# DJNing/articulated-object-nerf

Measured on AMD Instinct MI355X. Metric: rays/sec at 640×480×(64c+128f) samples; PSNR vs reference, higher is better.
Workload: dtype f16x3 (fp16 hi/lo split MFMA, fp32 accumulate)

## Files before the change

### articulated-object-nerf_amd/aonerf/_lib.py

```python
import ctypes
import os

import torch

_HERE = os.path.dirname(os.path.abspath(__file__))
LIB_PATH = os.path.join(os.path.dirname(_HERE), "lib", "libaonerf.so")

c_i64, c_int, c_float, c_size, vp = ctypes.c_int64, ctypes.c_int, ctypes.c_float, ctypes.c_size_t, ctypes.c_void_p

PREC = {"fp32": 0, "f16x3": 1}
PREC_F16X3_TRAIN = 4
PREC_BF16 = 2
ACT_NONE, ACT_VANILLA, ACT_ARTIC = 0, 1, 2
OPACITY = {None: 0, "mse": 1, "ce": 2, "autorf": 3}


class AonMlpParams(ctypes.Structure):
    _fields_ = [("pts_w", vp * 8), ("pts_b", vp * 8), ("density_w", vp), ("density_b", vp),
                ("bottleneck_w", vp), ("bottleneck_b", vp), ("views_w", vp), ("views_b", vp),
                ("rgb_w", vp), ("rgb_b", vp), ("w_rows", c_i64 * 12), ("w_cols", c_i64 * 12),
                ("b_len", c_i64 * 12)]


class AonMlpArtParams(ctypes.Structure):
# ... 123 lines not shown
    "aon_pos_enc": (c_int, [vp, c_i64, c_int, c_int, vp, vp]),
    "aon_sample_rays": (c_int, [vp, vp, c_int, c_i64, c_int, c_int, c_float, vp, c_i64, c_int,
                                c_float, vp, vp, vp, vp, vp]),
    "aon_cast_rays": (c_int, [vp, vp, vp, c_i64, c_int, vp, c_i64, vp, c_int, c_int, vp, vp]),
    "aon_cast_rays_tiled": (c_int, [vp, vp, vp, c_i64, c_int, c_int, c_int, c_int, vp, vp]),
    "aon_sample_pdf": (c_int, [vp, c_i64, vp, c_i64, c_i64, c_int, c_int, vp, c_i64, vp, c_int,
                               vp, vp, vp, vp, vp]),
    "aon_composite_march": (c_int, [vp, vp, vp, c_i64, c_int, c_int, c_int, vp, c_i64, c_int, vp,
                                    vp, vp, vp, vp, vp]),
    "aon_mlp_packed_bytes": (c_size, [c_int]),
    "aon_mlp_read_status": (c_int, [vp, c_size, ctypes.POINTER(ctypes.c_uint32), vp]),
    "aon_mlp_pack": (c_int, [ctypes.POINTER(AonMlpParams), c_int, vp, vp]),
    "aon_mlp_fwd": (c_int, [vp, c_int, vp, vp, vp, vp, c_i64, c_int, c_int, vp, vp]),
    "aon_mlp_fwd_encoded": (c_int, [vp, c_int, vp, vp, c_i64, c_int, c_int, vp, vp]),
    "aon_mlp_fwd_sigma": (c_int, [vp, c_int, vp, vp, vp, c_i64, c_int, c_int, vp, vp]),
    "aon_mlp_fwd_cond": (c_int, [vp, c_int, vp, vp, vp, vp, c_i64, c_int, c_int, vp, vp]),
    "aon_mlp_fwd_train": (c_int, [vp, vp, vp, vp, vp, c_i64, c_int, vp, vp, vp, vp, vp, vp, vp]),
    "aon_mlp_fwd_train_bf16": (c_int, [vp, vp, vp, vp, vp, c_i64, c_int, vp, vp, vp, vp, vp, vp,
                                       vp, vp]),
    "aon_mlp_bwd_pack_bf16": (c_int, [ctypes.POINTER(AonMlpParams), vp, vp]),
    "aon_mlp_bwd_bf16": (c_int, [vp, vp, vp, c_i64, vp, vp, vp, vp, vp]),
    "aon_relu_masks": (c_int, [vp, c_i64, c_int, vp, vp]),
    "aon_absmax": (c_int, [vp, c_i64, vp, vp]),
    "aon_mlp_bwd_packed_bytes": (c_size, []),
    "aon_mlp_bwd_pack": (c_int, [ctypes.POINTER(AonMlpParams), vp, vp]),
    "aon_mlp_bwd": (c_int, [vp, vp, vp, c_i64, vp, vp, vp, vp, vp]),
    "aon_mlp_art_packed_bytes": (c_size, []),
    "aon_mlp_art_pack": (c_int, [ctypes.POINTER(AonMlpArtParams), vp, vp]),
    "aon_mlp_art_fwd": (c_int, [vp, vp, vp, vp, vp, c_i64, c_int, c_int, vp, vp]),
    "aon_mlp_art_fwd_points": (c_int, [vp, vp, vp, c_i64, c_int, c_int, vp, vp]),
# ... 196 lines not shown
```

### articulated-object-nerf_amd/aonerf/model.py

```python
import warnings

import torch
import torch.nn as nn
import torch.nn.init as init

from . import _lib as L
from . import helper
from .numerics import resolve as _resolve_numerics

_DEFAULT_GEOMETRY = dict(min_deg_point=0, max_deg_point=10, deg_view=4, netdepth=8, netwidth=256,
                         netdepth_condition=1, netwidth_condition=128, skip_layer=4, input_ch=3,
                         input_ch_view=3, num_rgb_channels=3, num_density_channels=1)


class NeRFMLP(nn.Module):

    def __init__(self, min_deg_point, max_deg_point, deg_view, netdepth: int = 8,
                 netwidth: int = 256, netdepth_condition: int = 1, netwidth_condition: int = 128,
                 skip_layer: int = 4, input_ch: int = 3, input_ch_view: int = 3,
                 num_rgb_channels: int = 3, num_density_channels: int = 1,
                 precision: str = "f16x3"):
        super().__init__()
        self.min_deg_point, self.max_deg_point, self.deg_view = min_deg_point, max_deg_point, deg_view
        self.netdepth, self.netwidth, self.skip_layer = netdepth, netwidth, skip_layer
# ... 61 lines not shown
        L.require_gpu(rays_o, rays_d, viewdirs, t_vals, cond)
        B, S = t_vals.shape
        raw = torch.empty((B * S, 4), device=t_vals.device)
        if cond is not None:
            if tuple(cond.shape) != (B, 27):
                raise ValueError("forward_rays expects cond (B, 27)")
            L.call("aon_mlp_fwd_cond", L.ptr(self.packed_weights()), L.PREC[self.precision],
                   L.ptr(L.contig(rays_o)), L.ptr(L.contig(rays_d)), L.ptr(L.contig(cond)),
                   L.ptr(L.contig(t_vals)), B, S, act, L.ptr(raw), L.stream(t_vals.device))
            return raw
        L.call("aon_mlp_fwd", L.ptr(self.packed_weights()), L.PREC[self.precision],
               L.ptr(L.contig(rays_o)), L.ptr(L.contig(rays_d)), L.ptr(L.contig(viewdirs)),
               L.ptr(L.contig(t_vals)), B, S, act, L.ptr(raw), L.stream(t_vals.device))
        return raw

    def forward_sigma(self, rays_o, rays_d, t_vals, act=L.ACT_NONE):
        L.require_gpu(rays_o, rays_d, t_vals)
        B, S = t_vals.shape
        raw = torch.empty((B * S, 4), device=t_vals.device)
        L.call("aon_mlp_fwd_sigma", L.ptr(self.packed_weights()), L.PREC[self.precision],
               L.ptr(L.contig(rays_o)), L.ptr(L.contig(rays_d)), L.ptr(L.contig(t_vals)), B, S, act,
               L.ptr(raw), L.stream(t_vals.device))
        return raw

    def forward(self, x, condition):
        L.require_gpu(x, condition)
        B, S, C = x.shape
        if C != 63 or tuple(condition.shape) != (B, 27):
            raise ValueError("NeRFMLP.forward expects x (B, S, 63) and condition (B, 27)")
        raw = torch.empty((B * S, 4), device=x.device)
        L.call("aon_mlp_fwd_encoded", L.ptr(self.packed_weights()), L.PREC[self.precision],
               L.ptr(L.contig(x)), L.ptr(L.contig(condition)), B, S, L.ACT_NONE, L.ptr(raw),
               L.stream(x.device))
        raw = raw.view(B, S, 4)
        return raw[..., :3], raw[..., 3:]


# ... 19 lines not shown


def composite_march(raw, t_vals, d, white_bkgd, act, u, u_stride, num_fine_samples,
                    keep_weights):
    B, S = t_vals.shape
    dev = t_vals.device
    comp = torch.empty((B, 3), device=dev)
    acc = torch.empty((B,), device=dev)
    depth = torch.empty((B,), device=dev)
    weights = torch.empty((B, S), device=dev) if keep_weights else None
    t_fine = torch.empty((B, S + num_fine_samples), device=dev)
    L.call("aon_composite_march", L.ptr(raw), L.ptr(t_vals), L.ptr(d), B, S, int(bool(white_bkgd)),
           act, L.ptr(u), u_stride, num_fine_samples, L.ptr(comp), L.ptr(acc), L.ptr(weights),
           L.ptr(depth), L.ptr(t_fine), L.stream(dev))
    return (comp, acc, depth, weights), t_fine


def march_ok(S, num_fine_samples, fused=True):
    return fused and 3 <= S <= 256 and 1 <= num_fine_samples <= 256


def level_t_vals(level, o, d, t_prev, w_prev, randomized, near, far, num_coarse_samples,
                 num_fine_samples, lindisp, u_coarse=None, u_fine=None):
    dev = o.device
    B = o.shape[0]
    if level == 0:
        t_vals, _ = helper.sample_along_rays(o, d, num_coarse_samples, near, far, randomized,
                                             lindisp, u=u_coarse, want_coords=False)
        return t_vals
    Sc = t_prev.shape[1]
# ... 69 lines not shown
                comp, acc, depth, weights = RenderLevel.apply(o, d, v, t_vals, bool(white_bkgd),
                                                              noise, token, cfg, timers, *params)
                out = (comp, acc, depth, weights) if return_weights else (comp, acc, depth)
                if return_intermediates:
                    out = out + (dict(t_vals=t_vals, weights=weights),)
                ret.append(out)
                continue
            keep_w = level == 0 or return_weights or return_intermediates
            march = level == 0 and march_ok(S, self.num_fine_samples, self.fused_march)
            if march:
                keep_w = return_weights or return_intermediates
            with torch.no_grad():
                out, weights, t_next = self._render_level_fused(
                    mlp, o, d, v, t_vals, randomized, white_bkgd, level, timers, keep_w,
                    sigma_only=two_pass and level == 0, cond=cond if level == 1 else None,
                    march_u=(lambda: fine_uniforms(B, self.num_fine_samples, randomized, dev,
                                                   u_fine)) if march else None)
            if not return_weights:
                out = out[:3] + out[4:]
            if not return_intermediates:
                out = out[:4] if return_weights else out[:3]
            ret.append(None if fine_only and level == 0 else out)
        if (not training and self.range_check and self.coarse_mlp.precision.startswith("f16x3")
                and not torch.cuda.is_current_stream_capturing()
                and L.range_overflow([self.coarse_mlp._packed, self.fine_mlp._packed])):
            warnings.warn("NeRF: an MLP activation exceeded the fp16x3 range; re-rendered with "
                          "precision='fp32'", RuntimeWarning)
            prec = self.coarse_mlp.precision
            self.set_precision("fp32")
            if rng is not None:
# ... 1 lines not shown
            try:
                return self.forward(rays, randomized, white_bkgd, near, far, u_coarse=u_coarse,
                                    u_fine=u_fine, return_weights=return_weights,
                                    return_intermediates=return_intermediates, timers=timers,
                                    fine_only=fine_only)
            finally:
                self.set_precision(prec)
        return ret

    def _level_t(self, level, o, d, t_prev, w_prev, randomized, near, far, u_coarse, u_fine):
        return level_t_vals(level, o, d, t_prev, w_prev, randomized, near, far,
                            self.num_coarse_samples, self.num_fine_samples, self.lindisp,
                            u_coarse, u_fine)

    def _render_level_fused(self, mlp, o, d, v, t_vals, randomized, white_bkgd, level, timers,
                            keep_weights=True, march_u=None, sigma_only=False, cond=None):
        B, S = t_vals.shape
        dev = o.device
        noisy = self.noise_std > 0 and randomized
        ev = _events(timers)
        act = L.ACT_NONE if noisy else L.ACT_VANILLA
        if sigma_only:
            raw = mlp.forward_sigma(o, d, t_vals, act=act)
        else:
            raw = mlp.forward_rays(o, d, v, t_vals, act=act, cond=cond)
        _record(timers, ev, f"mlp{level}", B * S)
        if noisy:
            raw[:, 3] += torch.rand_like(raw[:, 3]) * self.noise_std
        act = L.ACT_VANILLA if noisy else L.ACT_NONE
        t_next = None
        ev = _events(timers)
        if march_u is not None:
            u, u_stride = march_u()
            (comp, acc, depth, weights), t_next = composite_march(
                raw, t_vals, d, white_bkgd, act, u, u_stride, self.num_fine_samples, keep_weights)
            _record(timers, ev, f"march{level}", B * S)
# ... 11 lines not shown
```

### articulated-object-nerf_amd/csrc/composite_core.hpp

```cpp
#pragma once

#include "aon_common.hpp"
#include "torch_sum.hpp"

namespace aon {

#ifndef AON_COMP_OCC_FINE
#define AON_COMP_OCC_FINE 6
#endif

constexpr int kCompWaves = 4;
constexpr int kCompMaxS = 512;
constexpr int kCompScratch = 256;

constexpr int comp_scratch(int S) {
  return S < 8 ? 256
               : 3 * 4 * ((S >> 2 >> 4) + 1) + 16 * 4 * (((S / 8) >> 2 >> 4) + 1);
}

__device__ __forceinline__ void wave_sync_c() {
  __builtin_amdgcn_fence(__ATOMIC_SEQ_CST, "wavefront");
  __builtin_amdgcn_wave_barrier();
}

template <int NB, int SC>
__device__ __forceinline__ void composite_ray(const float (&tt)[NB], const f4 (&raw)[NB],
                                              const float* __restrict__ dirs, int64_t ray, int S,
                                              int lane, int act, int white, float* P, int SM,
                                              float* scratch, float* sums,
                                              float* __restrict__ out_rgb,
                                              float* __restrict__ out_acc,
                                              float* __restrict__ out_w,
                                              float* __restrict__ out_depth) {
  const int64_t row0 = ray * S;
  const bool inner8 = S >= 8;
  const float dx = dirs[3 * ray], dy = dirs[3 * ray + 1], dz = dirs[3 * ray + 2];
  const float dnorm = sqrtf(fmaf(dz, dz, fmaf(dy, dy, __fmul_rn(dx, dx))));
  double carry = 1.0;
#pragma unroll
  for (int b = 0; b < NB; ++b) {
// ... 17 lines not shown
    const double incl = wave_incl_prod(f);
    const double excl = dpp_f64<0x138>(incl, 1.0);
    const float T = (float)(carry * excl);
    if (b + 1 < NB) carry *= readlane_f64(incl, 63);
    if (valid) {
      const float w = __fmul_rn(alpha, T);
      if (out_w) out_w[row0 + i] = w;
      P[i] = w;
      P[SM + i] = __fmul_rn(w, ti);
      P[2 * SM + i] = __fmul_rn(w, act_rgb(raw[b].x, act));
      P[3 * SM + i] = __fmul_rn(w, act_rgb(raw[b].y, act));
      P[4 * SM + i] = __fmul_rn(w, act_rgb(raw[b].z, act));
    }
  }
  wave_sync_c();
  wave_row_sums(
      [&](int sp, const float*& base, int& str) {
        if (sp < 3) {
          base = P + (2 + sp) * SM;
          str = 1;
        } else if (inner8) {
          base = P + ((sp - 3) >> 3) * SM + ((sp - 3) & 7);
          str = 8;
        } else {
          base = P + (sp - 3) * SM;
          str = 1;
        }
      },
      3, S, inner8 ? 16 : 2, inner8 ? S / 8 : S, scratch, sums, lane, wave_sync_c);
  if (lane < 2) {
// ... 29 lines not shown
```

### articulated-object-nerf_amd/csrc/march.hip

```cpp
#include "composite_core.hpp"
#include "pdf_core.hpp"

namespace aon {

template <int SM, int SCR, int NBX, int NO>
struct MarchLds {
  float P[5 * SM + SCR + 32];
  PdfLds<NBX> L;
  float orow[NO];
};

#ifndef AON_MARCH_OCC
#define AON_MARCH_OCC 7
#endif

template <int NB, int SC, int NBX>
__global__ __launch_bounds__(64 * kCompWaves, SC > 0 ? AON_MARCH_OCC : 1) void k_composite_march(
    const float* __restrict__ raw4, const float* __restrict__ tv, const float* __restrict__ dirs,
    int64_t B, int S_rt, int white, int act, const float* __restrict__ u_g, int64_t u_stride,
    int Ns, int Ns_pow2, float* __restrict__ out_rgb, float* __restrict__ out_acc,
    float* __restrict__ out_w, float* __restrict__ out_depth, float* __restrict__ t_out) {
  constexpr int SM = SC > 0 ? SC : 64 * NB;
  constexpr int kScratch = SC > 0 ? comp_scratch(SC) : kCompScratch;
  const int S = SC > 0 ? SC : S_rt;
  __shared__ MarchLds<SM, kScratch, NBX, SM + 64 * NBX> lds_all[kCompWaves];
  MarchLds<SM, kScratch, NBX, SM + 64 * NBX>& M = lds_all[threadIdx.x >> 6];
  float* P = M.P;
  float* scratch = P + 5 * SM;
  float* sums = scratch + kScratch;
  PdfLds<NBX>& L = M.L;
  const int lane = threadIdx.x & 63;
  const int nb = S - 1;
  const int64_t nwaves = (int64_t)gridDim.x * kCompWaves;
  for (int64_t ray = (int64_t)blockIdx.x * kCompWaves + (threadIdx.x >> 6); ray < B;
       ray += nwaves) {
    const int64_t row0 = ray * S;
    float tt[NB];
    f4 raw[NB];
#pragma unroll
    for (int b = 0; b < NB; ++b) {
      const int i = 64 * b + lane;
      tt[b] = 0.f;
      raw[b] = f4{0.f, 0.f, 0.f, 0.f};
      if (i < S) {
        tt[b] = tv[row0 + i];
        raw[b] = *reinterpret_cast<const f4*>(raw4 + (row0 + i) * 4);
      }
    }
    float cu[NBX];
#pragma unroll
    for (int b = 0; b < NBX; ++b) {
      const int i = 64 * b + lane;
      cu[b] = i < Ns ? u_g[ray * u_stride + i] : 0.f;
    }
#ifdef AON_MARCH_ABL_NOCOMP
#pragma unroll
    for (int b = 0; b < NB; ++b)
      if (64 * b + lane < S) P[64 * b + lane] = raw[b].w;
    wave_sync();
    if (false)
#endif
    composite_ray<NB, SC>(tt, raw, dirs, ray, S, lane, act, white, P, SM, scratch, sums, out_rgb,
                          out_acc, out_w, out_depth);
#pragma unroll
    for (int b = 0; b < NB; ++b) {
      const int i = 64 * b + lane;
      if (i < S) L.tm[i] = tt[b];
    }
    wave_sync();
    for (int k = lane; k < nb; k += 64) L.bins[k] = __fmul_rn(0.5f, __fadd_rn(L.tm[k + 1], L.tm[k]));
#ifndef AON_MARCH_ABL_NOPDF
    pdf_ray<NBX>(L, P + 1, nb, Ns, Ns_pow2, cu, true, S, ray, lane, M.orow, nullptr, nullptr,
                 nullptr);
#endif
    wave_sync();
    const int No = S + Ns;
    float* orow_g = t_out + ray * No;
    for (int i = lane; i < No; i += 64) orow_g[i] = M.orow[i];
// ... 72 lines not shown
struct WaveLds {
  RayLds r[4];
#if !AON_MARCH_DIRECT
  float orow[4 * kNo];
#endif
};

__device__ __forceinline__ int count_le64(const float* a, float x) {
  const bool all = a[63] <= x;
  int c = 0;
#pragma unroll
  for (int step = 32; step > 0; step >>= 1) c = a[c + step - 1] <= x ? c + step : c;
  return all ? 64 : c;
}

template <int ACT>
__global__ __launch_bounds__(64 * kWaves, AON_MARCH_ROWS_OCC) void k_march_rows(
    const float* __restrict__ raw4, const float* __restrict__ tv, const float* __restrict__ dirs,
    int64_t B, int white, const float* __restrict__ u_g, int64_t u_stride,
    float* __restrict__ out_rgb, float* __restrict__ out_acc, float* __restrict__ out_w,
    float* __restrict__ out_depth, float* __restrict__ t_out) {
  constexpr int act = ACT;
  __shared__ WaveLds lds_all[kWaves];
  WaveLds& WL = lds_all[threadIdx.x >> 6];
  const int lane = threadIdx.x & 63, row = lane >> 4, q = lane & 15;
  RayLds& L = WL.r[row];
  const int64_t ngroups = (B + 3) >> 2;
  const int64_t gstride = (int64_t)gridDim.x * kWaves;
  auto load_group = [&](int64_t g, float (&t5)[5], f4 (&r5)[5], float (&d3)[3]) {
    const int64_t ry = 4 * g + row;
    const uint32_t rr = static_cast<uint32_t>(ry < B ? ry : B - 1);
#pragma unroll
    for (int m = 0; m < 5; ++m) {
      const uint32_t i = rr * kS + (m < 4 ? 16 * m + q : 64);
      t5[m] = tv[i];
      r5[m] = *reinterpret_cast<const f4*>(raw4 + 4 * i);
    }
#pragma unroll
    for (int c = 0; c < 3; ++c) d3[c] = dirs[3 * rr + c];
  };
  int64_t grp = (int64_t)blockIdx.x * kWaves + (threadIdx.x >> 6);
  float ntt[5], nd[3];
  f4 nrw[5];
  if (AON_MARCH_PIPE && grp < ngroups) load_group(grp, ntt, nrw, nd);
  for (; grp < ngroups; grp += gstride) {
    const int64_t ray = 4 * grp + row;
    const bool valid = ray < B;
    const uint32_t rc = static_cast<uint32_t>(valid ? ray : B - 1);
    const uint32_t r0 = rc * kS;
    float tt[5], d3[3];
    f4 rw[5];
// ... 28 lines not shown
    const double e0 = row_bcast64<15>(hs[0]), e1 = row_bcast64<15>(hs[1]),
                 e2 = row_bcast64<15>(hs[2]);
    const double e01 = e1 * e0;
    double incl[4];
    incl[0] = hs[0];
    incl[1] = hs[1] * e0;
    incl[2] = hs[2] * e01;
    incl[3] = (hs[3] * e2) * e01;
    float w[5];
#pragma unroll
    for (int m = 0; m < 5; ++m) {
      const double sel = m == 4 ? incl[3] : (q == 15 ? (m == 0 ? 1.0 : incl[m - 1]) : incl[m]);
      const float T = (float)ror64<1>(sel);
      w[m] = __fmul_rn(alpha[m], T);
    }
    if (out_w && valid) {
#pragma unroll
      for (int m = 0; m < 5; ++m)
        if (m < 4 || q == 0) out_w[r0 + (m < 4 ? 16 * m + q : 64)] = w[m];
    }
    float rgb_out[3];
#pragma unroll
    for (int c = 0; c < 3; ++c) {
      float x[5];
#pragma unroll
      for (int m = 0; m < 5; ++m) x[m] = __fmul_rn(w[m], act_rgb(c == 0 ? rw[m].x : (c == 1 ? rw[m].y : rw[m].z), act));
      float acc = __fadd_rn(0.f, x[0]);
#pragma unroll
      for (int s = 1; s < 16; ++s) acc = __fadd_rn(ror<4>(acc), x[s >> 2]);
      float p = __fadd_rn(__fadd_rn(__fadd_rn(0.f, __fadd_rn(0.f, acc)), 0.f), 0.f);
      const float x64 = ror<12>(x[4]);
// ... 14 lines not shown
      for (int m = 0; m < 5; ++m) y[m] = v == 0 ? w[m] : __fmul_rn(w[m], tt[m]);
      const float a = __fadd_rn(__fadd_rn(0.f, y[0]), y[2]);
      const float b = __fadd_rn(__fadd_rn(0.f, y[1]), y[3]);
      const float part = __fadd_rn(__fadd_rn(__fadd_rn(a, ror<8>(a)), b), ror<8>(b));
      const float tail = ror<15>(__fadd_rn(0.f, y[4]));
      float s = q == 15 ? tail : part;
#pragma unroll
      for (int k = 0; k < 8; ++k) {
        const float nx = __fadd_rn(ror<1>(s), part);
        s = q == k ? nx : s;
      }
      sums2[v] = s;
    }
    {
      const float accv = ror<8>(sums2[0]);
      if (valid && q == 15) {
        float sr = rgb_out[0], sg = rgb_out[1], sb = rgb_out[2];
        if (white) {
          const float bg = __fsub_rn(1.0f, accv);
          sr = __fadd_rn(sr, bg);
          sg = __fadd_rn(sg, bg);
          sb = __fadd_rn(sb, bg);
        }
        out_rgb[3 * ray] = sr;
        out_rgb[3 * ray + 1] = sg;
        out_rgb[3 * ray + 2] = sb;
      }
      if (valid && q == 7) {
        out_acc[ray] = sums2[0];
        out_depth[ray] = nan_to_num(sums2[1], __builtin_inff());
      }
    }
#pragma unroll
    for (int m = 0; m < 4; ++m) {
      L.tm[16 * m + q] = tt[m];
      L.bins[16 * m + q] = __fmul_rn(0.5f, __fadd_rn(tn[m], tt[m]));
    }
    if (q == 0) L.tm[64] = tt[4];
    if (AON_MARCH_PIPE && grp + gstride < ngroups) load_group(grp + gstride, ntt, nrw, nd);
    float wn[4];
#pragma unroll
    for (int m = 0; m < 4; ++m) wn[m] = ror<15>(q == 0 ? w[m + 1] : w[m]);
    float ws;
// ... 217 lines not shown
    const int64_t nvalid = B - 4 * grp < 4 ? B - 4 * grp : 4;
    float* og = t_out + 4 * grp * kNo;
    const int n_out = static_cast<int>(nvalid) * kNo;
    for (int i = lane; i < n_out; i += 64) og[i] = WL.orow[i];
    wave_sync();
#endif
  }
}

}

#ifndef AON_MARCH_ROWS
#define AON_MARCH_ROWS 1
#endif

template <int NB, int SC, int NBX>
static void launch_march(hipStream_t st, const float* raw, const float* t, const float* dirs,
                         int64_t B, int S, int white, int act, const float* u, int64_t u_stride,
                         int Ns, int p2, float* comp, float* acc, float* w, float* depth,
                         float* t_out) {
  hipLaunchKernelGGL((k_composite_march<NB, SC, NBX>), grid_for(B, kCompWaves, 1 << 16),
                     64 * kCompWaves, 0, st, raw, t, dirs, B, S, white, act, u, u_stride, Ns, p2,
                     comp, acc, w, depth, t_out);
}

}

using namespace aon;

extern "C" int aon_composite_march(const float* raw, const float* t, const float* dirs, int64_t B,
                                   int S, int white_bkgd, int act, const float* u,
                                   int64_t u_stride, int Ns, float* comp_rgb, float* acc,
                                   float* weights, float* depth, float* t_fine,
                                   aon_stream_t stream) {
  AON_REQUIRE(raw && t && dirs && u && comp_rgb && acc && depth && t_fine, "null pointer");
  AON_REQUIRE(aligned16(raw), "raw must be a 16-byte aligned (B*S, 4) [r, g, b, sigma] array");
  AON_REQUIRE(B >= 0 && S >= 3 && S <= 256 && Ns >= 1 && Ns <= 256, "bad shape (3 <= S, Ns <= 256)");
  AON_REQUIRE(act >= AON_ACT_NONE && act <= AON_ACT_ARTIC, "bad activation");
  if (B == 0) return 0;
  int p2 = 1;
  while (p2 < Ns) p2 <<= 1;
  const int need = S > p2 ? S : p2;
  const int nbx = need <= 64 ? 1 : (need <= 128 ? 2 : 4);
  const int nb = (S + 63) / 64;
  hipStream_t st = (hipStream_t)stream;
#define AON_MARCH(NB_, SC_, NBX_)                                                                 \
  launch_march<NB_, SC_, NBX_>(st, raw, t, dirs, B, S, white_bkgd, act, u, u_stride, Ns, p2,      \
                               comp_rgb, acc, weights, depth, t_fine)
  if (AON_MARCH_ROWS && S == rowm::kS && Ns == rowm::kNs && B * rowm::kNo < (int64_t(1) << 31) &&
      (u_stride == 0 || B * u_stride < (int64_t(1) << 31))) {
    const int64_t groups = (B + 3) / 4;
#define AON_ROWS(A_)                                                                              \
  hipLaunchKernelGGL(rowm::k_march_rows<A_>,                                                      \
                     AON_MARCH_PIPE ? resident_grid(rowm::k_march_rows<A_>, 64 * rowm::kWaves,     \
                                                    (groups + rowm::kWaves - 1) / rowm::kWaves)    \
                                    : grid_for(groups, rowm::kWaves, 1 << 16),                     \
                     64 * rowm::kWaves, 0, st, raw, t, dirs, B, white_bkgd, u, u_stride, comp_rgb, \
                     acc, weights, depth, t_fine)
    if (act == AON_ACT_NONE) AON_ROWS(AON_ACT_NONE);
    else if (act == AON_ACT_VANILLA) AON_ROWS(AON_ACT_VANILLA);
    else AON_ROWS(AON_ACT_ARTIC);
#undef AON_ROWS
  } else if (S == 65 && nbx == 2) {
    AON_MARCH(2, 65, 2);
  } else {
#define AON_MARCH_NBX(NB_)                     \
  if (nbx == 1) AON_MARCH(NB_, 0, 1);          \
  else if (nbx == 2) AON_MARCH(NB_, 0, 2);     \
  else AON_MARCH(NB_, 0, 4);
    switch (nb) {
      case 1: AON_MARCH_NBX(1) break;
      case 2: AON_MARCH_NBX(2) break;
      case 3: AON_MARCH_NBX(3) break;
      default: AON_MARCH_NBX(4) break;
    }
#undef AON_MARCH_NBX
  }
#undef AON_MARCH
  return launch_status(__func__);
}
```

### articulated-object-nerf_amd/csrc/mlp.hip

```cpp
#include "aon_common.hpp"
#include "mlp_layout.hpp"
#include "mlp_pipe.hpp"
#include "param_check.hpp"

namespace aon {
namespace mlp {

constexpr int kWaves = 8;
constexpr int kThreads = 64 * kWaves;
constexpr int kRowsPerWave = 16;
constexpr int kRowsPerBlock = kRowsPerWave * kWaves;

__device__ __forceinline__ f4 mfma(float a, float b, f4 c) {
  return __builtin_amdgcn_mfma_f32_16x16x4f32(a, b, c, 0, 0, 0);
}

template <int LAYER, int NA, int NB, int NACC>
__device__ __forceinline__ void gemm(Pipe<kThreads>& p, const f4 (&xa)[NA], const f4 (&xb)[NB],
                                     f4 (&acc)[NACC]) {
  constexpr LayerDesc d = kLayers[LAYER];
  constexpr int U = d.u;
  static_assert(U % 4 == 0 && U <= NACC && d.ka <= NA && d.kb <= NB, "layer/array mismatch");
#pragma unroll
  for (int t = 0; t < d.ka + d.kb; ++t) {
// ... 320 lines not shown
  AON_REQUIRE(act >= AON_ACT_NONE && act <= AON_ACT_ARTIC, "bad activation");
  AON_REQUIRE(aligned16(packed) && aligned16(raw), "packed / raw must be 16-byte aligned");
  if (B * S == 0) return 1;
  AON_REQUIRE((B * S + 127) / 128 < (1ll << 31), "too many rows");
  return 0;
}

extern "C" int aon_mlp_fwd_sigma(const void* packed, int precision, const float* rays_o,
                                 const float* rays_d, const float* t, int64_t B, int S, int act,
                                 float* raw, aon_stream_t stream) {
  const int c = two_pass_check(packed, precision, rays_o, rays_d, t, B, S, act, raw);
  if (c) return c < 0 ? c : 0;
  return launch_f16x3_sigma(packed, rays_o, rays_d, t, B, S, act, raw, (hipStream_t)stream);
}

extern "C" int aon_mlp_fwd_cond(const void* packed, int precision, const float* rays_o,
                                const float* rays_d, const float* cond, const float* t, int64_t B,
                                int S, int act, float* raw, aon_stream_t stream) {
  AON_REQUIRE(cond, "null pointer");
  const int c = two_pass_check(packed, precision, rays_o, rays_d, t, B, S, act, raw);
  if (c) return c < 0 ? c : 0;
  return launch_f16x3_cond(packed, rays_o, rays_d, cond, t, B, S, act, raw, (hipStream_t)stream);
}

extern "C" int aon_mlp_fwd_train(const void* packed, const float* rays_o, const float* rays_d,
                                 const float* viewdirs, const float* t, int64_t B, int S,
                                 const float* noise, float* h, float* bot, float* hv, float* raw,
                                 uint32_t* masks, aon_stream_t stream) {
  AON_REQUIRE(packed && rays_o && rays_d && viewdirs && t && h && bot && hv && raw && masks,
              "null pointer");
// ... 33 lines not shown
```

### articulated-object-nerf_amd/csrc/mlp_f16x3.hip

```cpp
#include "mlp_f16x3_core.hpp"

namespace aon {
namespace mlp {

#ifndef AON_STASH_REGS
#define AON_STASH_REGS 0
#endif

#ifndef AON_STAGGER
#define AON_STAGGER 0
#endif

template <bool BF, bool SIG = false>
__host__ __device__ constexpr int stash_per() { return BF ? 3 : (SIG ? 4 : 6); }
template <bool BF, bool SIG = false>
__device__ __forceinline__ int enc_slot(int c, int k, int lo) {
  return BF ? 3 * c + k : stash_per<BF, SIG>() * c + 2 * k + lo;
}
template <bool BF>
__device__ __forceinline__ int venc_slot(int c, int lo) { return BF ? 3 * c + 2 : 6 * c + 4 + lo; }

template <typename Net>
constexpr bool kSigmaOnly = std::is_same<Net, NetVanillaSigmaH>::value;
static_assert(kStreamBlocksSigma % kChunkH == 0 &&
// ... 68 lines not shown
        f4 o = {0.0f, 0.0f, 0.0f, act_sigma(sig, act)};
        if constexpr (!SIG) {
          o[0] = act_rgb(rgb[c][0] * s, act);
          o[1] = act_rgb(rgb[c][1] * s, act);
          o[2] = act_rgb(rgb[c][2] * s, act);
        }
#ifdef AON_ABL_NO_RAW_STORE
        if (__builtin_isnan(o[0] + o[1] + o[2] + o[3]))
#endif
        *reinterpret_cast<f4*>(raw + 4 * rows[c]) = o;
      }
    }
  }
}

template <int MODE, int NCOL, bool STORE = false, bool BF = false, typename Net = NetVanillaH>
__global__ __launch_bounds__((GeomH<NCOL, BF>::kThreads), (GeomH<NCOL, BF>::kWavesPerSimd)) void k_mlp_fwd_f16x3(
    const f4* __restrict__ wstream, const float* __restrict__ bias_g, const float* __restrict__ in0,
    const float* __restrict__ in1, const float* __restrict__ in2, const float* __restrict__ in3,
    int64_t B, int S, int act, float* __restrict__ raw, TrainStore ts = {}) {
  using G = GeomH<NCOL, BF>;
  constexpr bool SIG = kSigmaOnly<Net>;
  static_assert(!SIG || MODE == 0, "the density-only pass takes MODE 0 inputs");
  constexpr int kPer = stash_per<BF, SIG>() * NCOL;
  constexpr int kStash = AON_STASH_REGS ? 0 : G::kWaves * 64 * kPer;
  static_assert((kLdsWeights + Net::kBiasFloats / 4 + kStash) * 16 <= 160 * 1024, "LDS");
  __shared__ f4 smem[kLdsWeights + Net::kBiasFloats / 4 + kStash];
  float* bias_s = reinterpret_cast<float*>(smem + kLdsWeights);
  f4* stash = smem + kLdsWeights + Net::kBiasFloats / 4 + (threadIdx.x >> 6) * 64 * kPer +
              (threadIdx.x & 63);

  const int tid = threadIdx.x, lane = tid & 63, wave = tid >> 6;
  const int g = lane >> 4, j = lane & 15;
  const int64_t N = B * S;

  WeightPipeP<Net, G::kThreads, BF> p;
  p.wbuf = smem;
  p.src = wstream;
  p.tid = tid;
  p.lane = lane;
  p.start();
  for (int i = tid; i < Net::kBiasFloats; i += G::kThreads) bias_s[i] = bias_g[i];

  Frag<2, NCOL> enc;
  Frag<1, NCOL> venc;
  int64_t rows[NCOL];
#pragma unroll
  for (int c = 0; c < NCOL; ++c) {
    const int64_t row = (int64_t)blockIdx.x * G::kRowsPerBlock + wave * G::kRowsPerWave + 16 * c + j;
    rows[c] = row;
    const int64_t rr = row < N ? row : N - 1;
    const int64_t ray = rr / S;
    float ev[2][8], vv[8];
    if constexpr (MODE == 0 && !SIG) {
      const float* ro = in0 + 3 * ray;
      const float* rd = in1 + 3 * ray;
      const float* vd = in2 + 3 * ray;
      const float tt = in3[rr];
      const float x0 = __fadd_rn(ro[0], __fmul_rn(tt, rd[0]));
      const float x1 = __fadd_rn(ro[1], __fmul_rn(tt, rd[1]));
      const float x2 = __fadd_rn(ro[2], __fmul_rn(tt, rd[2]));
      const float v0 = vd[0], v1 = vd[1], v2 = vd[2];
      auto encode = [&](auto fast) {
#pragma unroll
        for (int k = 0; k < 2; ++k)
#pragma unroll
          for (int e = 0; e < 8; ++e)
// ... 278 lines not shown
  return reinterpret_cast<const float*>(static_cast<const char*>(packed) +
                                        NetVanillaFoldH::kStreamBytes);
}

int launch_f16x3_sigma(const void* packed, const float* rays_o, const float* rays_d,
                       const float* t, int64_t B, int S, int act, float* raw, hipStream_t stream) {
  using G = GeomH<1>;
  const int64_t N = B * S;
  hipLaunchKernelGGL((k_mlp_fwd_f16x3<0, 1, false, false, NetVanillaSigmaH>),
                     static_cast<int>((N + G::kRowsPerBlock - 1) / G::kRowsPerBlock), G::kThreads, 0,
                     stream, static_cast<const f4*>(packed), fold_bias(packed), rays_o, rays_d,
                     static_cast<const float*>(nullptr), t, B, S, act, raw);
  return launch_status("aon_mlp_fwd_sigma");
}

int launch_f16x3_cond(const void* packed, const float* rays_o, const float* rays_d,
                      const float* cond, const float* t, int64_t B, int S, int act, float* raw,
                      hipStream_t stream) {
  using G = GeomH<1>;
  const int64_t N = B * S;
  hipLaunchKernelGGL((k_mlp_fwd_f16x3<2, 1, false, false, NetVanillaFoldH>),
                     static_cast<int>((N + G::kRowsPerBlock - 1) / G::kRowsPerBlock), G::kThreads, 0,
                     stream, static_cast<const f4*>(packed), fold_bias(packed), rays_o, rays_d, cond,
                     t, B, S, act, raw);
  return launch_status("aon_mlp_fwd_cond");
}

}
}
```

### articulated-object-nerf_amd/csrc/mlp_layout.hpp

```cpp
#pragma once

namespace aon {
namespace mlp {

struct LayerDesc {
  int ka, kb;
  int u;
  int len_a, len_b;
  int out_real;
  int blk0;
  int bias0;
};

enum { L0 = 0, L1, L2, L3, L4, L5, L6, L7, LDEN, LBOT, LVIEW, LRGB, kNumLayers };

constexpr int kChunk = 16;

constexpr LayerDesc kLayers[kNumLayers] = {
    {4, 0, 16, 63, 0, 256, 0, 0},
    {16, 0, 16, 256, 0, 256, 64, 256},
    {16, 0, 16, 256, 0, 256, 320, 512},
    {16, 0, 16, 256, 0, 256, 576, 768},
    {16, 0, 16, 256, 0, 256, 832, 1024},
    {16, 4, 16, 256, 63, 256, 1088, 1280},
// ... 314 lines not shown
  __bf16* enc_bf;
};

int pack_f16x3(const PackArgs& a, void* packed, hipStream_t stream, bool bf16 = false,
               bool fold = false);
int pack_h(PackArgsH a, void* packed, hipStream_t stream);
int absmax(const float* x, int64_t n, uint32_t* out, hipStream_t stream);
int launch_f16x3(int mode, int ncol, const void* packed, const float* a0, const float* a1,
                 const float* a2, const float* a3, int64_t B, int S, int act, float* raw,
                 hipStream_t stream, const TrainStore* ts = nullptr);
int launch_f16x3_sigma(const void* packed, const float* rays_o, const float* rays_d,
                       const float* t, int64_t B, int S, int act, float* raw, hipStream_t stream);
int launch_f16x3_cond(const void* packed, const float* rays_o, const float* rays_d,
                      const float* cond, const float* t, int64_t B, int S, int act, float* raw,
                      hipStream_t stream);
#ifndef AON_DATAFLOW_WS_BUILD
#define AON_DATAFLOW_WS_BUILD 0
#endif
int launch_ws_f16x3(const void* packed, const float* a0, const float* a1, const float* a2,
                    const float* a3, int64_t B, int S, int act, float* raw, hipStream_t stream);
int launch_art_ws_f16x3(const void* packed, const float* a0, const float* a1, const float* a2,
                        const float* a3, int64_t B, int S, int act, float* raw, hipStream_t stream);

}
}
```

### include/aonerf.h

```cpp
#ifndef AONERF_H
#define AONERF_H

#include <stddef.h>
#include <stdint.h>

#ifdef __cplusplus
extern "C" {
#endif

typedef void* aon_stream_t;

#define AON_ABI_VERSION 13

#define AON_PREC_FP32 0
#define AON_PREC_F16X3 1
#define AON_PREC_F16X3_TRAIN 4
#define AON_PREC_BF16 2

#define AON_ACT_NONE 0
#define AON_ACT_VANILLA 1
#define AON_ACT_ARTIC 2

int aon_abi_version(void);
const char* aon_last_error(void);
// ... 46 lines not shown
int aon_cast_rays_tiled(const float* rays_o, const float* rays_d, const float* t, int64_t B, int S,
                        int min_deg, int max_deg, int width, float* enc, aon_stream_t stream);

int aon_pos_enc(const float* x, int64_t n, int min_deg, int max_deg, float* out,
                aon_stream_t stream);

int aon_sample_pdf(const float* bins, int64_t bins_stride, const float* weights,
                   int64_t w_stride, int64_t B, int nb, int Ns, const float* u,
                   int64_t u_stride, const float* t_merge, int Nt, const float* rays_o,
                   const float* rays_d, float* out, float* xyz, aon_stream_t stream);

int aon_composite_march(const float* raw, const float* t, const float* dirs, int64_t B, int S,
                        int white_bkgd, int act, const float* u, int64_t u_stride, int Ns,
                        float* comp_rgb, float* acc, float* weights, float* depth, float* t_fine,
                        aon_stream_t stream);

typedef struct aon_mlp_params {
  const float* pts_w[8];
  const float* pts_b[8];
  const float* density_w;
  const float* density_b;
  const float* bottleneck_w;
  const float* bottleneck_b;
  const float* views_w;
  const float* views_b;
  const float* rgb_w;
  const float* rgb_b;
  int64_t w_rows[12], w_cols[12], b_len[12];
} aon_mlp_params;

// ... 3 lines not shown

int aon_mlp_read_status(const void* packed, size_t packed_bytes, uint32_t* status,
                        aon_stream_t stream);

int aon_mlp_fwd(const void* packed, int precision, const float* rays_o, const float* rays_d,
                const float* viewdirs, const float* t, int64_t B, int S, int act, float* out,
                aon_stream_t stream);


int aon_mlp_fwd_encoded(const void* packed, int precision, const float* x,
                        const float* condition, int64_t B, int S, int act, float* out,
                        aon_stream_t stream);

int aon_mlp_fwd_sigma(const void* packed, int precision, const float* rays_o, const float* rays_d,
                      const float* t, int64_t B, int S, int act, float* out, aon_stream_t stream);

int aon_mlp_fwd_cond(const void* packed, int precision, const float* rays_o, const float* rays_d,
                     const float* cond, const float* t, int64_t B, int S, int act, float* out,
                     aon_stream_t stream);

int aon_mlp_fwd_train(const void* packed, const float* rays_o, const float* rays_d,
                      const float* viewdirs, const float* t, int64_t B, int S, const float* noise,
                      float* h, float* bot, float* hv, float* raw, uint32_t* masks,
                      aon_stream_t stream);

int aon_mlp_fwd_train_bf16(const void* packed, const float* rays_o, const float* rays_d,
                           const float* viewdirs, const float* t, int64_t B, int S,
                           const float* noise, uint16_t* h, uint16_t* bot, uint16_t* hv,
                           float* raw, uint32_t* masks, uint16_t* enc, aon_stream_t stream);

// ... 175 lines not shown
```

Measured before the change: 1.685 million.

## Skip last coarse sample and unused outputs in the two-pass coarse density march

In the two-pass coarse level, the density MLP now evaluates only the first S-1 samples of each ray, since the last sample's density does not affect the weights used for importance sampling. The composite march gets a HEAD variant that zeroes the last sample's raw value and skips writing rgb, acc, depth and weights, producing only the fine sample positions. This saves one of 64 coarse MLP evaluations per ray plus the coarse output stores. In exchange it adds template variants and a remapped row indexing in the MLP kernel, and the coarse outputs are no longer available on this path.

After: 1.690 million, median of 6. About the same (+0.3%).

```diff
diff --git a/articulated-object-nerf_amd/aonerf/_lib.py b/articulated-object-nerf_amd/aonerf/_lib.py
--- a/articulated-object-nerf_amd/aonerf/_lib.py
+++ b/articulated-object-nerf_amd/aonerf/_lib.py
@@ -161,6 +161,8 @@
     "aon_mlp_fwd": (c_int, [vp, c_int, vp, vp, vp, vp, c_i64, c_int, c_int, vp, vp]),
     "aon_mlp_fwd_encoded": (c_int, [vp, c_int, vp, vp, c_i64, c_int, c_int, vp, vp]),
     "aon_mlp_fwd_sigma": (c_int, [vp, c_int, vp, vp, vp, c_i64, c_int, c_int, vp, vp]),
+    "aon_mlp_fwd_sigma_head": (c_int, [vp, c_int, vp, vp, vp, c_i64, c_int, c_int, c_int, vp, vp]),
+    "aon_composite_march_head": (c_int, [vp, vp, vp, c_i64, c_int, c_int, vp, c_i64, c_int, vp, vp]),
     "aon_mlp_fwd_cond": (c_int, [vp, c_int, vp, vp, vp, vp, c_i64, c_int, c_int, vp, vp]),
     "aon_mlp_fwd_train": (c_int, [vp, vp, vp, vp, vp, c_i64, c_int, vp, vp, vp, vp, vp, vp, vp]),
     "aon_mlp_fwd_train_bf16": (c_int, [vp, vp, vp, vp, vp, c_i64, c_int, vp, vp, vp, vp, vp, vp,
diff --git a/articulated-object-nerf_amd/aonerf/model.py b/articulated-object-nerf_amd/aonerf/model.py
--- a/articulated-object-nerf_amd/aonerf/model.py
+++ b/articulated-object-nerf_amd/aonerf/model.py
@@ -99,13 +99,16 @@
                L.ptr(L.contig(t_vals)), B, S, act, L.ptr(raw), L.stream(t_vals.device))
         return raw
 
-    def forward_sigma(self, rays_o, rays_d, t_vals, act=L.ACT_NONE):
+    def forward_sigma(self, rays_o, rays_d, t_vals, act=L.ACT_NONE, head=False):
         L.require_gpu(rays_o, rays_d, t_vals)
         B, S = t_vals.shape
         raw = torch.empty((B * S, 4), device=t_vals.device)
-        L.call("aon_mlp_fwd_sigma", L.ptr(self.packed_weights()), L.PREC[self.precision],
-               L.ptr(L.contig(rays_o)), L.ptr(L.contig(rays_d)), L.ptr(L.contig(t_vals)), B, S, act,
-               L.ptr(raw), L.stream(t_vals.device))
+        args = (L.ptr(self.packed_weights()), L.PREC[self.precision], L.ptr(L.contig(rays_o)),
+                L.ptr(L.contig(rays_d)), L.ptr(L.contig(t_vals)), B, S)
+        if head:
+            L.call("aon_mlp_fwd_sigma_head", *args, S - 1, act, L.ptr(raw), L.stream(t_vals.device))
+        else:
+            L.call("aon_mlp_fwd_sigma", *args, act, L.ptr(raw), L.stream(t_vals.device))
         return raw
 
     def forward(self, x, condition):
@@ -155,6 +158,14 @@
            act, L.ptr(u), u_stride, num_fine_samples, L.ptr(comp), L.ptr(acc), L.ptr(weights),
            L.ptr(depth), L.ptr(t_fine), L.stream(dev))
     return (comp, acc, depth, weights), t_fine
+
+
+def composite_march_head(raw, t_vals, d, act, u, u_stride, num_fine_samples):
+    B, S = t_vals.shape
+    t_fine = torch.empty((B, S + num_fine_samples), device=t_vals.device)
+    L.call("aon_composite_march_head", L.ptr(raw), L.ptr(t_vals), L.ptr(d), B, S, act, L.ptr(u),
+           u_stride, num_fine_samples, L.ptr(t_fine), L.stream(t_vals.device))
+    return t_fine
 
 
 def march_ok(S, num_fine_samples, fused=True):
@@ -254,6 +265,7 @@
                 out, weights, t_next = self._render_level_fused(
                     mlp, o, d, v, t_vals, randomized, white_bkgd, level, timers, keep_w,
                     sigma_only=two_pass and level == 0, cond=cond if level == 1 else None,
+                    head=two_pass and march and not (self.noise_std > 0 and randomized),
                     march_u=(lambda: fine_uniforms(B, self.num_fine_samples, randomized, dev,
                                                    u_fine)) if march else None)
             if not return_weights:
@@ -285,12 +297,23 @@
                             u_coarse, u_fine)
 
     def _render_level_fused(self, mlp, o, d, v, t_vals, randomized, white_bkgd, level, timers,
-                            keep_weights=True, march_u=None, sigma_only=False, cond=None):
+                            keep_weights=True, march_u=None, sigma_only=False, cond=None,
+                            head=False):
         B, S = t_vals.shape
         dev = o.device
         noisy = self.noise_std > 0 and randomized
         ev = _events(timers)
         act = L.ACT_NONE if noisy else L.ACT_VANILLA
+        if head:
+            assert sigma_only and march_u is not None and not noisy
+            raw = mlp.forward_sigma(o, d, t_vals, act=act, head=True)
+            _record(timers, ev, f"mlp{level}", B * S)
+            ev = _events(timers)
+            u, u_stride = march_u()
+            t_next = composite_march_head(raw, t_vals, d, L.ACT_NONE, u, u_stride,
+                                          self.num_fine_samples)
+            _record(timers, ev, f"march{level}", B * S)
+            return (None, None, None, None, None), None, t_next
         if sigma_only:
             raw = mlp.forward_sigma(o, d, t_vals, act=act)
         else:
diff --git a/articulated-object-nerf_amd/csrc/composite_core.hpp b/articulated-object-nerf_amd/csrc/composite_core.hpp
--- a/articulated-object-nerf_amd/csrc/composite_core.hpp
+++ b/articulated-object-nerf_amd/csrc/composite_core.hpp
@@ -23,7 +23,7 @@
   __builtin_amdgcn_wave_barrier();
 }
 
-template <int NB, int SC>
+template <int NB, int SC, bool OUT = true>
 __device__ __forceinline__ void composite_ray(const float (&tt)[NB], const f4 (&raw)[NB],
                                               const float* __restrict__ dirs, int64_t ray, int S,
                                               int lane, int act, int white, float* P, int SM,
@@ -71,6 +71,7 @@
     }
   }
   wave_sync_c();
+  if constexpr (!OUT) return;
   wave_row_sums(
       [&](int sp, const float*& base, int& str) {
         if (sp < 3) {
diff --git a/articulated-object-nerf_amd/csrc/march.hip b/articulated-object-nerf_amd/csrc/march.hip
--- a/articulated-object-nerf_amd/csrc/march.hip
+++ b/articulated-object-nerf_amd/csrc/march.hip
@@ -14,7 +14,7 @@
 #define AON_MARCH_OCC 7
 #endif
 
-template <int NB, int SC, int NBX>
+template <int NB, int SC, int NBX, bool HEAD = false>
 __global__ __launch_bounds__(64 * kCompWaves, SC > 0 ? AON_MARCH_OCC : 1) void k_composite_march(
     const float* __restrict__ raw4, const float* __restrict__ tv, const float* __restrict__ dirs,
     int64_t B, int S_rt, int white, int act, const float* __restrict__ u_g, int64_t u_stride,
@@ -44,7 +44,7 @@
       raw[b] = f4{0.f, 0.f, 0.f, 0.f};
       if (i < S) {
         tt[b] = tv[row0 + i];
-        raw[b] = *reinterpret_cast<const f4*>(raw4 + (row0 + i) * 4);
+        if (!HEAD || i < S - 1) raw[b] = *reinterpret_cast<const f4*>(raw4 + (row0 + i) * 4);
       }
     }
     float cu[NBX];
@@ -60,8 +60,8 @@
     wave_sync();
     if (false)
 #endif
-    composite_ray<NB, SC>(tt, raw, dirs, ray, S, lane, act, white, P, SM, scratch, sums, out_rgb,
-                          out_acc, out_w, out_depth);
+    composite_ray<NB, SC, !HEAD>(tt, raw, dirs, ray, S, lane, act, white, P, SM, scratch, sums,
+                                 out_rgb, out_acc, out_w, out_depth);
 #pragma unroll
     for (int b = 0; b < NB; ++b) {
       const int i = 64 * b + lane;
@@ -164,7 +164,7 @@
   return all ? 64 : c;
 }
 
-template <int ACT>
+template <int ACT, bool HEAD = false>
 __global__ __launch_bounds__(64 * kWaves, AON_MARCH_ROWS_OCC) void k_march_rows(
     const float* __restrict__ raw4, const float* __restrict__ tv, const float* __restrict__ dirs,
     int64_t B, int white, const float* __restrict__ u_g, int64_t u_stride,
@@ -184,7 +184,8 @@
     for (int m = 0; m < 5; ++m) {
       const uint32_t i = rr * kS + (m < 4 ? 16 * m + q : 64);
       t5[m] = tv[i];
-      r5[m] = *reinterpret_cast<const f4*>(raw4 + 4 * i);
+      if (HEAD && m == 4) r5[m] = f4{0.f, 0.f, 0.f, 0.f};
+      else r5[m] = *reinterpret_cast<const f4*>(raw4 + 4 * i);
     }
 #pragma unroll
     for (int c = 0; c < 3; ++c) d3[c] = dirs[3 * rr + c];
@@ -243,7 +244,7 @@
       const float T = (float)ror64<1>(sel);
       w[m] = __fmul_rn(alpha[m], T);
     }
-    if (out_w && valid) {
+    if (!HEAD && out_w && valid) {
 #pragma unroll
       for (int m = 0; m < 5; ++m)
         if (m < 4 || q == 0) out_w[r0 + (m < 4 ? 16 * m + q : 64)] = w[m];
@@ -288,7 +289,7 @@
     }
     {
       const float accv = ror<8>(sums2[0]);
-      if (valid && q == 15) {
+      if (!HEAD && valid && q == 15) {
         float sr = rgb_out[0], sg = rgb_out[1], sb = rgb_out[2];
         if (white) {
           const float bg = __fsub_rn(1.0f, accv);
@@ -300,7 +301,7 @@
         out_rgb[3 * ray + 1] = sg;
         out_rgb[3 * ray + 2] = sb;
       }
-      if (valid && q == 7) {
+      if (!HEAD && valid && q == 7) {
         out_acc[ray] = sums2[0];
         out_depth[ray] = nan_to_num(sums2[1], __builtin_inff());
       }
@@ -548,30 +549,21 @@
 #define AON_MARCH_ROWS 1
 #endif
 
-template <int NB, int SC, int NBX>
+template <int NB, int SC, int NBX, bool HEAD>
 static void launch_march(hipStream_t st, const float* raw, const float* t, const float* dirs,
                          int64_t B, int S, int white, int act, const float* u, int64_t u_stride,
                          int Ns, int p2, float* comp, float* acc, float* w, float* depth,
                          float* t_out) {
-  hipLaunchKernelGGL((k_composite_march<NB, SC, NBX>), grid_for(B, kCompWaves, 1 << 16),
+  hipLaunchKernelGGL((k_composite_march<NB, SC, NBX, HEAD>), grid_for(B, kCompWaves, 1 << 16),
                      64 * kCompWaves, 0, st, raw, t, dirs, B, S, white, act, u, u_stride, Ns, p2,
                      comp, acc, w, depth, t_out);
 }
 
-}
-
-using namespace aon;
-
-extern "C" int aon_composite_march(const float* raw, const float* t, const float* dirs, int64_t B,
-                                   int S, int white_bkgd, int act, const float* u,
-                                   int64_t u_stride, int Ns, float* comp_rgb, float* acc,
-                                   float* weights, float* depth, float* t_fine,
-                                   aon_stream_t stream) {
-  AON_REQUIRE(raw && t && dirs && u && comp_rgb && acc && depth && t_fine, "null pointer");
-  AON_REQUIRE(aligned16(raw), "raw must be a 16-byte aligned (B*S, 4) [r, g, b, sigma] array");
-  AON_REQUIRE(B >= 0 && S >= 3 && S <= 256 && Ns >= 1 && Ns <= 256, "bad shape (3 <= S, Ns <= 256)");
-  AON_REQUIRE(act >= AON_ACT_NONE && act <= AON_ACT_ARTIC, "bad activation");
-  if (B == 0) return 0;
+template <bool HEAD>
+static int march_dispatch(const char* fn, const float* raw, const float* t, const float* dirs,
+                          int64_t B, int S, int white_bkgd, int act, const float* u,
+                          int64_t u_stride, int Ns, float* comp_rgb, float* acc, float* weights,
+                          float* depth, float* t_fine, aon_stream_t stream) {
   int p2 = 1;
   while (p2 < Ns) p2 <<= 1;
   const int need = S > p2 ? S : p2;
@@ -579,14 +571,14 @@
   const int nb = (S + 63) / 64;
   hipStream_t st = (hipStream_t)stream;
 #define AON_MARCH(NB_, SC_, NBX_)                                                                 \
-  launch_march<NB_, SC_, NBX_>(st, raw, t, dirs, B, S, white_bkgd, act, u, u_stride, Ns, p2,      \
+  launch_march<NB_, SC_, NBX_, HEAD>(st, raw, t, dirs, B, S, white_bkgd, act, u, u_stride, Ns, p2,      \
                                comp_rgb, acc, weights, depth, t_fine)
   if (AON_MARCH_ROWS && S == rowm::kS && Ns == rowm::kNs && B * rowm::kNo < (int64_t(1) << 31) &&
       (u_stride == 0 || B * u_stride < (int64_t(1) << 31))) {
     const int64_t groups = (B + 3) / 4;
 #define AON_ROWS(A_)                                                                              \
-  hipLaunchKernelGGL(rowm::k_march_rows<A_>,                                                      \
-                     AON_MARCH_PIPE ? resident_grid(rowm::k_march_rows<A_>, 64 * rowm::kWaves,     \
+  hipLaunchKernelGGL((rowm::k_march_rows<A_, HEAD>),                                              \
+                     AON_MARCH_PIPE ? resident_grid(rowm::k_march_rows<A_, HEAD>, 64 * rowm::kWaves, \
                                                     (groups + rowm::kWaves - 1) / rowm::kWaves)    \
                                     : grid_for(groups, rowm::kWaves, 1 << 16),                     \
                      64 * rowm::kWaves, 0, st, raw, t, dirs, B, white_bkgd, u, u_stride, comp_rgb, \
@@ -611,5 +603,36 @@
 #undef AON_MARCH_NBX
   }
 #undef AON_MARCH
-  return launch_status(__func__);
-}
+  return launch_status(fn);
+}
+
+}
+
+using namespace aon;
+
+extern "C" int aon_composite_march(const float* raw, const float* t, const float* dirs, int64_t B,
+                                   int S, int white_bkgd, int act, const float* u,
+                                   int64_t u_stride, int Ns, float* comp_rgb, float* acc,
+                                   float* weights, float* depth, float* t_fine,
+                                   aon_stream_t stream) {
+  AON_REQUIRE(raw && t && dirs && u && comp_rgb && acc && depth && t_fine, "null pointer");
+  AON_REQUIRE(aligned16(raw), "raw must be a 16-byte aligned (B*S, 4) [r, g, b, sigma] array");
+  AON_REQUIRE(B >= 0 && S >= 3 && S <= 256 && Ns >= 1 && Ns <= 256, "bad shape (3 <= S, Ns <= 256)");
+  AON_REQUIRE(act >= AON_ACT_NONE && act <= AON_ACT_ARTIC, "bad activation");
+  if (B == 0) return 0;
+  return march_dispatch<false>(__func__, raw, t, dirs, B, S, white_bkgd, act, u, u_stride, Ns,
+                               comp_rgb, acc, weights, depth, t_fine, stream);
+}
+
+extern "C" int aon_composite_march_head(const float* raw, const float* t, const float* dirs,
+                                        int64_t B, int S, int act, const float* u,
+                                        int64_t u_stride, int Ns, float* t_fine,
+                                        aon_stream_t stream) {
+  AON_REQUIRE(raw && t && dirs && u && t_fine, "null pointer");
+  AON_REQUIRE(aligned16(raw), "raw must be a 16-byte aligned (B*S, 4) [r, g, b, sigma] array");
+  AON_REQUIRE(B >= 0 && S >= 3 && S <= 256 && Ns >= 1 && Ns <= 256, "bad shape (3 <= S, Ns <= 256)");
+  AON_REQUIRE(act >= AON_ACT_NONE && act <= AON_ACT_ARTIC, "bad activation");
+  if (B == 0) return 0;
+  return march_dispatch<true>(__func__, raw, t, dirs, B, S, 0, act, u, u_stride, Ns, nullptr,
+                              nullptr, nullptr, nullptr, t_fine, stream);
+}
diff --git a/articulated-object-nerf_amd/csrc/mlp.hip b/articulated-object-nerf_amd/csrc/mlp.hip
--- a/articulated-object-nerf_amd/csrc/mlp.hip
+++ b/articulated-object-nerf_amd/csrc/mlp.hip
@@ -358,6 +358,17 @@
   return launch_f16x3_sigma(packed, rays_o, rays_d, t, B, S, act, raw, (hipStream_t)stream);
 }
 
+extern "C" int aon_mlp_fwd_sigma_head(const void* packed, int precision, const float* rays_o,
+                                      const float* rays_d, const float* t, int64_t B, int S,
+                                      int S_eval, int act, float* raw, aon_stream_t stream) {
+  const int c = two_pass_check(packed, precision, rays_o, rays_d, t, B, S, act, raw);
+  if (c < 0) return c;
+  AON_REQUIRE(S_eval >= 1 && S_eval <= S, "bad shape (1 <= S_eval <= S)");
+  if (c) return 0;
+  return launch_f16x3_sigma_head(packed, rays_o, rays_d, t, B, S, S_eval, act, raw,
+                                 (hipStream_t)stream);
+}
+
 extern "C" int aon_mlp_fwd_cond(const void* packed, int precision, const float* rays_o,
                                 const float* rays_d, const float* cond, const float* t, int64_t B,
                                 int S, int act, float* raw, aon_stream_t stream) {
diff --git a/articulated-object-nerf_amd/csrc/mlp_f16x3.hip b/articulated-object-nerf_amd/csrc/mlp_f16x3.hip
--- a/articulated-object-nerf_amd/csrc/mlp_f16x3.hip
+++ b/articulated-object-nerf_amd/csrc/mlp_f16x3.hip
@@ -106,14 +106,16 @@
   }
 }
 
-template <int MODE, int NCOL, bool STORE = false, bool BF = false, typename Net = NetVanillaH>
+template <int MODE, int NCOL, bool STORE = false, bool BF = false, typename Net = NetVanillaH,
+          bool HEAD = false>
 __global__ __launch_bounds__((GeomH<NCOL, BF>::kThreads), (GeomH<NCOL, BF>::kWavesPerSimd)) void k_mlp_fwd_f16x3(
     const f4* __restrict__ wstream, const float* __restrict__ bias_g, const float* __restrict__ in0,
     const float* __restrict__ in1, const float* __restrict__ in2, const float* __restrict__ in3,
-    int64_t B, int S, int act, float* __restrict__ raw, TrainStore ts = {}) {
+    int64_t B, int S, int act, float* __restrict__ raw, TrainStore ts = {}, int S_eval = 0) {
   using G = GeomH<NCOL, BF>;
   constexpr bool SIG = kSigmaOnly<Net>;
   static_assert(!SIG || MODE == 0, "the density-only pass takes MODE 0 inputs");
+  static_assert(!HEAD || SIG, "only the density-only pass stops short of a ray's last sample");
   constexpr int kPer = stash_per<BF, SIG>() * NCOL;
   constexpr int kStash = AON_STASH_REGS ? 0 : G::kWaves * 64 * kPer;
   static_assert((kLdsWeights + Net::kBiasFloats / 4 + kStash) * 16 <= 160 * 1024, "LDS");
@@ -125,6 +127,7 @@
   const int tid = threadIdx.x, lane = tid & 63, wave = tid >> 6;
   const int g = lane >> 4, j = lane & 15;
   const int64_t N = B * S;
+  const int64_t NR = HEAD ? B * S_eval : N;
 
   WeightPipeP<Net, G::kThreads, BF> p;
   p.wbuf = smem;
@@ -140,9 +143,10 @@
 #pragma unroll
   for (int c = 0; c < NCOL; ++c) {
     const int64_t row = (int64_t)blockIdx.x * G::kRowsPerBlock + wave * G::kRowsPerWave + 16 * c + j;
-    rows[c] = row;
-    const int64_t rr = row < N ? row : N - 1;
-    const int64_t ray = rr / S;
+    const int64_t rp = row < NR ? row : NR - 1;
+    const int64_t ray = rp / (HEAD ? S_eval : S);
+    const int64_t rr = HEAD ? ray * S + (rp - ray * S_eval) : rp;
+    rows[c] = HEAD ? (row < NR ? rr : N) : row;
     float ev[2][8], vv[8];
     if constexpr (MODE == 0 && !SIG) {
       const float* ro = in0 + 3 * ray;
@@ -451,6 +455,18 @@
   return launch_status("aon_mlp_fwd_sigma");
 }
 
+int launch_f16x3_sigma_head(const void* packed, const float* rays_o, const float* rays_d,
+                            const float* t, int64_t B, int S, int S_eval, int act, float* raw,
+                            hipStream_t stream) {
+  using G = GeomH<1>;
+  const int64_t NR = B * S_eval;
+  hipLaunchKernelGGL((k_mlp_fwd_f16x3<0, 1, false, false, NetVanillaSigmaH, true>),
+                     static_cast<int>((NR + G::kRowsPerBlock - 1) / G::kRowsPerBlock), G::kThreads, 0,
+                     stream, static_cast<const f4*>(packed), fold_bias(packed), rays_o, rays_d,
+                     static_cast<const float*>(nullptr), t, B, S, act, raw, TrainStore{}, S_eval);
+  return launch_status("aon_mlp_fwd_sigma_head");
+}
+
 int launch_f16x3_cond(const void* packed, const float* rays_o, const float* rays_d,
                       const float* cond, const float* t, int64_t B, int S, int act, float* raw,
                       hipStream_t stream) {
diff --git a/articulated-object-nerf_amd/csrc/mlp_layout.hpp b/articulated-object-nerf_amd/csrc/mlp_layout.hpp
--- a/articulated-object-nerf_amd/csrc/mlp_layout.hpp
+++ b/articulated-object-nerf_amd/csrc/mlp_layout.hpp
@@ -352,6 +352,9 @@
 int launch_f16x3_cond(const void* packed, const float* rays_o, const float* rays_d,
                       const float* cond, const float* t, int64_t B, int S, int act, float* raw,
                       hipStream_t stream);
+int launch_f16x3_sigma_head(const void* packed, const float* rays_o, const float* rays_d,
+                            const float* t, int64_t B, int S, int S_eval, int act, float* raw,
+                            hipStream_t stream);
 #ifndef AON_DATAFLOW_WS_BUILD
 #define AON_DATAFLOW_WS_BUILD 0
 #endif
diff --git a/include/aonerf.h b/include/aonerf.h
--- a/include/aonerf.h
+++ b/include/aonerf.h
@@ -84,6 +84,10 @@
                         int white_bkgd, int act, const float* u, int64_t u_stride, int Ns,
                         float* comp_rgb, float* acc, float* weights, float* depth, float* t_fine,
                         aon_stream_t stream);
+
+int aon_composite_march_head(const float* raw, const float* t, const float* dirs, int64_t B,
+                             int S, int act, const float* u, int64_t u_stride, int Ns,
+                             float* t_fine, aon_stream_t stream);
 
 typedef struct aon_mlp_params {
   const float* pts_w[8];
@@ -117,6 +121,10 @@
 
 int aon_mlp_fwd_sigma(const void* packed, int precision, const float* rays_o, const float* rays_d,
                       const float* t, int64_t B, int S, int act, float* out, aon_stream_t stream);
+
+int aon_mlp_fwd_sigma_head(const void* packed, int precision, const float* rays_o,
+                           const float* rays_d, const float* t, int64_t B, int S, int S_eval,
+                           int act, float* out, aon_stream_t stream);
 
 int aon_mlp_fwd_cond(const void* packed, int precision, const float* rays_o, const float* rays_d,
                      const float* cond, const float* t, int64_t B, int S, int act, float* out,
```
